# LUMC/kPAL

Hardware: AMD Instinct MI355X
Metric: Gbases/s k-mer counted (k=12, 150bp synthetic) (higher is better)
Workload: dtype int64

## Files before the change

### include/kpal_hip.h

```cpp
#ifndef KPAL_HIP_H
#define KPAL_HIP_H

#include <stddef.h>
#include <stdint.h>

#ifdef __cplusplus
extern "C" {
#endif

#define KPAL_MAX_K 16

#define KPAL_OK 0
#define KPAL_E_INVALID (-1)
#define KPAL_E_NOMEM (-2)
#define KPAL_E_HIP (-3)
#define KPAL_E_STATE (-4)
#define KPAL_E_IO (-5)

#define KPAL_PAIRWISE_PROD 0
#define KPAL_PAIRWISE_SUM 1
#define KPAL_EUCLIDEAN 2

#define KPAL_COSINE 3

// ... 45 lines not shown
int kpal_fastq_flatten(kpal_ctx *ctx, const uint8_t *host_buf, size_t nbytes, const kpal_fastq_options *opt, uint8_t *host_out,
                       uint64_t *n_out);
int kpal_count_records(kpal_ctx *ctx, int k, const uint8_t *host_flat, size_t nbytes, const uint64_t *host_starts,
                       size_t n_records, int64_t *host_out);
int kpal_fasta_records_begin(kpal_ctx *ctx, const uint8_t *host_text, size_t nbytes, uint64_t *n_records, uint64_t *flat_bytes);
int kpal_fasta_records_index(kpal_ctx *ctx, uint64_t *header_off, uint64_t *flat_start);
int kpal_fasta_records_count(kpal_ctx *ctx, int k, uint64_t first, uint64_t n, int64_t *host_out);
int kpal_fasta_records_count_device(kpal_ctx *ctx, int k, uint64_t first, uint64_t n, int64_t *dev_out);
int kpal_fasta_records_file_open(kpal_ctx *ctx, const char *path, uint64_t begin, uint64_t end);
int kpal_fasta_records_file_next(kpal_ctx *ctx, uint64_t *n_records, uint64_t *flat_bytes, uint64_t *text_offset, int *done);
int kpal_fasta_records_file_tell(kpal_ctx *ctx, uint64_t *offset);
int kpal_fasta_records_file_close(kpal_ctx *ctx);
int kpal_count_finish(kpal_ctx *ctx, int64_t *host_out );
int kpal_count_balance(kpal_ctx *ctx);
int kpal_count_last_plan(kpal_ctx *ctx, int *strategy, int *steps1, int *steps2);
#define KPAL_COUNT_STATS 9
int kpal_count_stats(kpal_ctx *ctx, uint64_t *out, int n);
int kpal_count_table(kpal_ctx *ctx, void **dev_table, uint64_t *n_bins);

int kpal_synth_reads_device(kpal_ctx *ctx, uint64_t seed, uint64_t first_read, uint64_t n_reads,
                            int read_len, int noisy, void *dev_out);

#define KPAL_COMM_ID_BYTES 128
int kpal_comm_probe(const char *rccl_library);
int kpal_comm_unique_id(const char *rccl_library, uint8_t *id_out );
int kpal_comm_init(kpal_ctx *ctx, const char *rccl_library, int rank, int world, const uint8_t *id);
int kpal_comm_destroy(kpal_ctx *ctx);
int kpal_comm_reduce_table(kpal_ctx *ctx, int root, int balance);
int kpal_comm_reduce_table_async(kpal_ctx *ctx, int root, int balance);
int kpal_comm_merged_table(kpal_ctx *ctx, void **dev_table, uint64_t *n_bins);
int kpal_comm_reduce_scatter_table(kpal_ctx *ctx, int balance);
// ... 94 lines not shown
```

### kpal_amd/_native.py

```python
import ctypes
import os
import numbers
import threading

import numpy as np

_HERE = os.path.dirname(os.path.abspath(__file__))
LIB_PATH = os.environ.get('KPAL_HIP_LIBRARY', os.path.join(_HERE, 'libkpal_hip.so'))

KPAL_MAX_K = 16
PAIRWISE_PROD, PAIRWISE_SUM, EUCLIDEAN, COSINE = 0, 1, 2, 3
SUMMARY_MIN, SUMMARY_AVERAGE, SUMMARY_MEDIAN = 0, 1, 2
STRATEGY = {'auto': 0, 'global_atomic': 1, 'lds_direct': 2, 'partition': 3, 'partition2': 4, 'partition_chunked': 5, 'partition_quads': 6, 'partition2_quads': 7}

_E_INVALID, _E_NOMEM, _E_HIP, _E_STATE, _E_IO = -1, -2, -3, -4, -5

_lib = None
_lib_lock = threading.Lock()

_vp = ctypes.c_void_p
_i64p = ctypes.POINTER(ctypes.c_int64)
_f64p = ctypes.POINTER(ctypes.c_double)

class DistanceOptions(ctypes.Structure):
# ... 359 lines not shown
        p = _vp()
        n = ctypes.c_uint64(0)
        _check(self._L.kpal_count_table(self._h, ctypes.byref(p), ctypes.byref(n)))
        return p.value, n.value

    def count_balance(self):
        _check(self._L.kpal_count_balance(self._h))

    def count_last_plan(self):
        st, s1, s2 = ctypes.c_int(0), ctypes.c_int(0), ctypes.c_int(0)
        _check(self._L.kpal_count_last_plan(self._h, ctypes.byref(st), ctypes.byref(s1), ctypes.byref(s2)))
        names = {v: n for n, v in STRATEGY.items()}
        return names.get(st.value, str(st.value)), s1.value, s2.value

    def count_stats(self):
        out = (ctypes.c_uint64 * 9)()
        _check(self._L.kpal_count_stats(self._h, out, 9))
        names = ('hot_entries', 'spilled_items', 'unlisted_items', 'fresh_pieces', 'fresh_reruns', 'quad_pieces', 'chunked_pieces', 'split_pieces', 'repeat_pieces')
        return dict(zip(names, (int(v) for v in out)))

    def count_table_view(self):
        ptr, n = self.count_table()
        return DeviceTable(ptr, n, self)

    def synth_reads_device(self, seed, first_read, n_reads, read_len, dev_ptr, noisy=False):
        _check(self._L.kpal_synth_reads_device(self._h, int(seed), int(first_read), int(n_reads), int(read_len),
                                               int(bool(noisy)), _vp(dev_ptr)))

    def count_records(self, k, flat, starts):
        a = np.frombuffer(flat, dtype=np.uint8) if not isinstance(flat, np.ndarray) else np.ascontiguousarray(flat, dtype=np.uint8)
        st = np.ascontiguousarray(starts, dtype=np.uint64)
        n = st.size - 1
        out = np.empty((max(n, 0), 4 ** k), dtype=np.int64)
# ... 312 lines not shown
```

### kpal_amd/csrc/kpal_count.hip

```cpp
#include "kpal_host.hpp"

#include "count_kernels.hpp"
#include "partition_kernels.hpp"
#include "chunk_kernels.hpp"
#include "fasta_kernels.hpp"
#include "fasta_host.hpp"
#include "fastq_kernels.hpp"

#include <cerrno>
#include <fcntl.h>
#include <sys/stat.h>
#include <sys/syscall.h>
#include <unistd.h>

static_assert(sizeof(ChunkPool) <= sizeof(kpal_ctx::chunk_pool_sent), "kpal_ctx::chunk_pool_sent holds a ChunkPool");

static void fq_reset(kpal_ctx *ctx);

KPAL_API int kpal_count_begin(kpal_ctx *ctx, int k)
{
    CTX_ENTER(ctx);
    if (k < 1 || k > KPAL_MAX_K) return set_err(KPAL_E_INVALID, "k=%d out of range 1..%d", k, KPAL_MAX_K);
    if (ctx->merged && (ctx->merged_bins != (1ULL << (2 * k)) || ctx->merged == ctx->table.p)) {
        ctx->merged = nullptr;
// ... 1230 lines not shown
    if (steps1) *steps1 = ctx->plan_steps1;
    if (steps2) *steps2 = ctx->plan_steps2;
    return KPAL_OK;
}

KPAL_API int kpal_count_stats(kpal_ctx *ctx, uint64_t *out, int n)
{
    CTX_ENTER(ctx);
    if (!out || n < 1) return set_err(KPAL_E_INVALID, "out is NULL");
    uint32_t words[4] = {0, 0, 0, 0};
    if (ctx->quad_error_word) {
        HIPCHK(hipMemcpyAsync(words, ctx->quad_error_word, sizeof(words), hipMemcpyDeviceToHost, ctx->stream));
        HIPCHK(hipStreamSynchronize(ctx->stream));
    }
    const uint64_t all[KPAL_COUNT_STATS] = {words[1], words[2], words[3], ctx->stat_fresh_pieces, ctx->stat_fresh_reruns, ctx->stat_quad_pieces,
                                            ctx->stat_chunked_pieces, ctx->stat_split_pieces, ctx->stat_repeat_pieces};
    for (int i = 0; i < n; ++i) out[i] = i < KPAL_COUNT_STATS ? all[i] : 0;
    return KPAL_OK;
}

KPAL_API int kpal_count_table(kpal_ctx *ctx, void **dev_table, uint64_t *n_bins)
{
    if (!ctx) return set_err(KPAL_E_INVALID, "ctx is NULL");
    if (!ctx->counting) return set_err(KPAL_E_STATE, "no count table (call kpal_count_begin)");
    HIPCHK(hipSetDevice(ctx->device));
    CHK(table_ready(ctx));
    if (dev_table) *dev_table = ctx->table.p;
    if (n_bins) *n_bins = ctx->bins;
    return KPAL_OK;
}

// ... 16 lines not shown
```

### kpal_amd/csrc/kpal_ctx.hip

```cpp
#include "kpal_host.hpp"

#include <unistd.h>

static thread_local char g_err[512] = "";

int set_err(int code, const char *fmt, ...)
{
    va_list ap;
    va_start(ap, fmt);
    vsnprintf(g_err, sizeof(g_err), fmt, ap);
    va_end(ap);
    return code;
}

KPAL_API const char *kpal_last_error(void) { return g_err; }
KPAL_API const char *kpal_version(void) { return "kpal_amd 0.4 (gfx950)"; }

int ensure(kpal_ctx *ctx, DevBuf &b, size_t bytes)
{
    if (b.cap >= bytes && b.p) return KPAL_OK;
    if (b.p) {
        HIPCHK(hipStreamSynchronize(ctx->stream));
        HIPCHK(hipFree(b.p));
        b.p = nullptr;
// ... 89 lines not shown
    }
    if (const char *e = getenv("KPAL_BATCH_BYTES")) {
        unsigned long long v = strtoull(e, nullptr, 10);
        if (v >= (1ULL << 20)) {
            ctx->batch_bytes = (size_t)v;
            ctx->batch_bytes_set = true;
        }
    }
    if (const char *e = getenv("KPAL_LEVEL2")) ctx->level2_mode = atoi(e);
    if (const char *e = getenv("KPAL_FASTA_CHUNK")) {
        const unsigned long long v = strtoull(e, nullptr, 10);
        if (v >= 16 && v <= kpal_ctx::kStage) ctx->fa_chunk = (size_t)v;
    }
    if (const char *e = getenv("KPAL_QUAD_STEPS")) ctx->quad_steps_forced = atoi(e);
    if (const char *e = getenv("KPAL_QUAD_STEPS2")) ctx->quad_steps2_forced = atoi(e);
    if (const char *e = getenv("KPAL_QUAD_VERBOSE")) ctx->quad_verbose = atoi(e) != 0;
    if (const char *e = getenv("KPAL_QUAD_REPEAT")) ctx->quad_repeat_forced = atoi(e) != 0 ? 1 : 0;
    if (const char *e = getenv("KPAL_HIST_PACKED")) ctx->quad_hist_unpacked = atoi(e) == 0;
    if (const char *e = getenv("KPAL_DIRECT_SEG")) {
        const long v = atol(e);
        if (v >= 1 && v <= (1 << 20)) {
            ctx->direct_seg = (uint32_t)v;
            ctx->direct_seg_forced = true;
        }
    }
    if (const char *e = getenv("KPAL_SPLIT_ABOVE")) {
        unsigned long long v = strtoull(e, nullptr, 10);
        if (v >= 1024) ctx->split_above = v;
    }
    if (const char *e = getenv("KPAL_QUAD_POOL_MAX")) {
// ... 160 lines not shown
```

### kpal_amd/csrc/kpal_device.hpp

```cpp
#pragma once
#include <hip/hip_runtime.h>
#include <stdint.h>

namespace kpal {

__host__ __device__ inline uint64_t mix64(uint64_t x)
{
    uint64_t z = x + 0x9E3779B97F4A7C15ULL;
    z = (z ^ (z >> 30)) * 0xBF58476D1CE4E5B9ULL;
    z = (z ^ (z >> 27)) * 0x94D049BB133111EBULL;
    return z ^ (z >> 31);
}

__host__ __device__ inline uint64_t revcomp(uint64_t x, int k)
{
    uint64_t y = ~x;
#if defined(__HIP_DEVICE_COMPILE__)
    y = __brevll(y);
#else
    y = ((y >> 1) & 0x5555555555555555ULL) | ((y & 0x5555555555555555ULL) << 1);
    y = ((y >> 2) & 0x3333333333333333ULL) | ((y & 0x3333333333333333ULL) << 2);
    y = ((y >> 4) & 0x0F0F0F0F0F0F0F0FULL) | ((y & 0x0F0F0F0F0F0F0F0FULL) << 4);
    y = ((y >> 8) & 0x00FF00FF00FF00FFULL) | ((y & 0x00FF00FF00FF00FFULL) << 8);
    y = ((y >> 16) & 0x0000FFFF0000FFFFULL) | ((y & 0x0000FFFF0000FFFFULL) << 16);
// ... 174 lines not shown
                                            uint64_t &window, uint32_t &mask, bool edge)
{
    const int lane = threadIdx.x & 63;
    const int64_t c = (int64_t)(step * 64 + lane);
    Chunk cur = encode16(raw);
    if (edge) range_fix(s, c, cur);
    const uint32_t pc = from_left_lane(cur.codes, carry.codes);
    const uint32_t pb = from_left_lane(cur.bad, carry.bad);
    carry.codes = __builtin_amdgcn_readlane(cur.codes, 63);
    carry.bad = __builtin_amdgcn_readlane(cur.bad, 63);
    window = ((uint64_t)pc << 32) | cur.codes;
    mask = emit_mask<K>(pb, cur.bad);
    if (edge) mask &= emit_from_mask(s, c);
}

__device__ __forceinline__ bool interior_steps(const Span &s, uint64_t step0, uint64_t step1)
{
    return step0 * 64 >= 1 && (step0 * 64 - 1) * 16 >= s.lo && step1 * 64 * 16 <= s.hi && s.emit_from <= step0 * 64 * 16;
}

template <int K>
__device__ __forceinline__ void encode_step(const Span &s, uint64_t step, const uint4 raw, Chunk &carry,
                                            uint64_t &window, uint32_t &mask)
{
    encode_step<K>(s, step, raw, carry, window, mask, !interior_steps(s, step, step + 1));
}

__device__ __forceinline__ bool interior_range(const Span &s, uint64_t c0, uint64_t c1)
{
    return c0 >= 1 && (c0 - 1) * 16 >= s.lo && c1 * 16 <= s.hi && s.emit_from <= c0 * 16;
// ... 24 lines not shown
```

### kpal_amd/csrc/kpal_host.hpp

```cpp
#pragma once
#include "../../include/kpal_hip.h"

#include <hip/hip_runtime.h>

#include <algorithm>
#include <cmath>
#include <cstdarg>
#include <cstdio>
#include <cstdlib>
#include <cstring>
#include <string>
#include <thread>
#include <type_traits>
#include <vector>

#include "kpal_device.hpp"
#include "host_pool.hpp"

#define KPAL_API extern "C" __attribute__((visibility("default")))

using namespace kpal;

int set_err(int code, const char *fmt, ...) __attribute__((format(printf, 2, 3)));

// ... 32 lines not shown
    int strategy = KPAL_STRATEGY_AUTO;
    bool counting = false;
    DevBuf table;
    uint64_t bins = 0;
    size_t batch_bytes = (size_t)1 << 30;
    bool batch_bytes_set = false;
    uint64_t split_above = 0xFFFFFFFFull;
    size_t quad_pool_max = (size_t)30 << 30;
    DevBuf keys, cntmat, offs, bucket_start, slice_start;
    DevBuf chunk_meta, chunk_table, chunk_ovf, chunk_sorted;
    DevBuf quad_meta, quad_meta2;
    uint32_t *quad_error_word = nullptr;
    bool chunk_error_armed = false;
    int quad_steps_forced = 0, quad_steps2_forced = 0;
    bool quad_verbose = false;
    int quad_repeat_forced = -1;
    bool sample_hot_rows = false;
    int plan_strategy = 0, plan_steps1 = 0, plan_steps2 = 0;
    uint64_t stat_fresh_pieces = 0, stat_fresh_reruns = 0, stat_quad_pieces = 0, stat_chunked_pieces = 0, stat_split_pieces = 0, stat_repeat_pieces = 0;
    int cached_steps1 = 0, cached_steps2 = 0;
    uint32_t cached_uses = 0;
    size_t cached_bytes = 0;
    bool finalize_pending = false;
    const void *finalize_stage = nullptr;
    bool table_zero_pending = false;
    bool finalize_fresh = false;
    bool fresh_resolved = false;
    bool fresh_feed = false;
    Span fresh_span = {};
    DevBuf direct_list, direct_meta;
    uint32_t direct_seg = 16384;
    uint32_t direct_seg_used = 16384;
    bool quad_hist_unpacked = false;
// ... 190 lines not shown
```

### kpal_amd/csrc/kpal_quads.hip

```cpp
#include "kpal_host.hpp"

#include "quad_kernels.hpp"


double quad_expected_backlog(const std::vector<double> &mu, int slots)
{
    static const double rho_grid[10] = {0.5, 0.6, 0.7, 0.75, 0.8, 0.85, 0.9, 0.925, 0.95, 0.975};
    static const double ratio[4][10] = {
        {1.02, 1.08, 1.25, 1.43, 1.70, 2.19, 3.21, 4.24, 6.34, 12.7},
        {1.00, 1.01, 1.08, 1.17, 1.33, 1.65, 2.34, 3.05, 4.52, 8.9},
        {1.00, 1.00, 1.01, 1.04, 1.12, 1.30, 1.75, 2.24, 3.25, 6.35},
        {1.00, 1.00, 1.00, 1.02, 1.02, 1.10, 1.36, 1.68, 2.37, 4.55}};
    const int ti = slots <= 24 ? 0 : (slots <= 32 ? 1 : (slots <= 64 ? 2 : 3));
    double total = 0.0;
    for (size_t at = 0; at < mu.size();) {
        size_t end = at + 1;
        while (end < mu.size() && mu[end] <= mu[at] * 1.01) ++end;
        const double m = 0.5 * (mu[at] + mu[end - 1]), weight = (double)(end - at);
        at = end;
        if (m <= 0.0) continue;
        const double rho = m / slots;
        if (rho >= 0.995) {
            total += 1e6 * weight;
            continue;
// ... 69 lines not shown
        for (size_t b = 0; b < mu.size(); ++b) mu[b] = per_step[b] * waves * c;
        const double backlog = quad_expected_backlog(mu, slots);
        if (verbose) fprintf(stderr, "[kpal quad] sample: %d steps per wave -> expected backlog %.0f items (fullest row %.1f of %d)\n", c, backlog, mu.back(), slots);
        if (backlog <= budget) {
            *steps_out = c;
            break;
        }
    }
    return KPAL_OK;
}

int launch_partition_quads(kpal_ctx *ctx, const Span &s)
{
    const uint64_t total_steps = (s.nchunks + 63) / 64;
    if (total_steps == 0) return KPAL_OK;
    const int buckets = ctx->k == 12 ? QuadCfg<12>::kBuckets : 512;
    const int slots = ctx->k == 12 ? QuadCfg<12>::kItems : kQuadRowWords / buckets;
    CHK(ensure(ctx, ctx->quad_meta, ((size_t)ctx->num_cu + 4 + 2048 + 512) * sizeof(uint32_t)));
    uint32_t *nrounds = (uint32_t *)ctx->quad_meta.p;
    uint32_t *error = nrounds + ctx->num_cu;
    uint32_t *load = error + 4;
    if (!ctx->quad_error_word) {
        HIPCHK(hipMemsetAsync(error, 0, 4 * sizeof(uint32_t), ctx->stream));
        ctx->quad_error_word = error;
    }
    static const int candidates[] = {8, 7, 6, 4, 3, 2, 1};
    constexpr int waves = 16;
    int steps = 0;
    for (int c : candidates)
        if (c == ctx->quad_steps_forced) steps = c;
// ... 8 lines not shown
        const int rc = quad_choose_steps(ctx, s, load, buckets, slots, waves, candidates, sizeof(candidates) / sizeof(candidates[0]), &steps);
        if (rc != KPAL_OK) return rc;
        repeat = ctx->sample_hot_rows;
        ctx->cached_steps1 = steps;
        ctx->cached_uses = 0;
        ctx->cached_bytes = feed_bytes;
    }
    if (ctx->quad_repeat_forced >= 0) repeat = ctx->quad_repeat_forced != 0;
    if (repeat && steps == 7 && !ctx->quad_steps_forced) steps = 6;
    if (repeat && steps != 7) ++ctx->stat_repeat_pieces;
    ctx->plan_strategy = KPAL_STRATEGY_PARTITION_QUADS;
    ctx->plan_steps1 = steps;
    ctx->plan_steps2 = 0;
    const uint64_t tile_steps = (uint64_t)waves * steps;
    const uint64_t tiles = (total_steps + tile_steps - 1) / tile_steps;
    const uint32_t G = (uint32_t)std::min<uint64_t>((uint64_t)ctx->num_cu, tiles);
    const uint64_t tpb = (tiles + G - 1) / G;
    if (tpb > 0xFFFFFFull) return set_err(KPAL_E_INVALID, "quad partition: batch too large");
    const size_t pool_bytes = (size_t)kQuadRowWords * 4 * G * tpb;
    if (pool_bytes > ctx->quad_pool_max && s.nchunks > 64) return kSplitBatch;
    CHK(ensure(ctx, ctx->keys, pool_bytes));
    uint32_t *pool = (uint32_t *)ctx->keys.p;
    const TableOnly table = {(unsigned long long *)ctx->table.p};
    static const bool allow_staged = [] { const char *e = getenv("KPAL_K12_STAGED"); return !e || atoi(e) != 0; }();
    uint32_t *stage = nullptr;
    if (ctx->k == 12 && allow_staged && (double)feed_bytes <= 240.0 * 4.0 * (double)ctx->bins) {
        CHK(ensure(ctx, ctx->residuals, (size_t)ctx->bins * 4 * sizeof(quad2_stage_t)));
        stage = (uint32_t *)ctx->residuals.p;
    }
#define KPAL_QUAD_LAUNCH(S)                                                                                                  \
    do {                                                                                                                     \
        if (repeat)                                                                                                          \
// ... 37 lines not shown
```

### kpal_amd/csrc/kpal_quads2.hip

```cpp
#include "kpal_host.hpp"

#include "quad_kernels.hpp"

#ifndef KPAL_L1_DEPTH8
#define KPAL_L1_DEPTH8 4
#endif

int launch_partition2_quads(kpal_ctx *ctx, const Span &s, bool fresh)
{
    const uint64_t total_steps = (s.nchunks + 63) / 64;
    if (total_steps == 0) return KPAL_OK;
    const int K = ctx->k;
    const uint32_t NB1 = 1u << (2 * K - 22);
    const uint32_t REP = NB1 >= 256 ? 1u : 256u / NB1;
    const uint32_t S1 = (uint32_t)kQuadRowWords / (NB1 * REP);
    CHK(ensure(ctx, ctx->quad_meta, ((size_t)ctx->num_cu + 4 + 2048 + 512) * sizeof(uint32_t)));
    uint32_t *nrounds1 = (uint32_t *)ctx->quad_meta.p;
    uint32_t *error = nrounds1 + ctx->num_cu;
    if (!ctx->quad_error_word) {
        HIPCHK(hipMemsetAsync(error, 0, 4 * sizeof(uint32_t), ctx->stream));
        ctx->quad_error_word = error;
    }
    static const int candidates[] = {8, 7, 6, 3};
    int steps1 = 0;
    for (int c : candidates)
        if (c == ctx->quad_steps_forced) steps1 = c;
// ... 2 lines not shown
    const bool cached = ctx->cached_steps1 && ctx->cached_steps2 && ctx->cached_uses < 16 && feed_bytes <= 2 * ctx->cached_bytes &&
                        2 * feed_bytes >= ctx->cached_bytes;
    if (cached) {
        if (!steps1) steps1 = ctx->cached_steps1;
        ++ctx->cached_uses;
    } else {
        int chosen = 0;
        const int rc = quad_choose_steps(ctx, s, error + 4, (int)(NB1 * REP), (int)S1, 16, candidates, 4, &chosen, &fine);
        if (rc != KPAL_OK) return rc;
        if (!steps1) steps1 = chosen;
    }
    const bool repeat1 = ctx->quad_repeat_forced >= 0 ? ctx->quad_repeat_forced != 0 : ctx->sample_hot_rows;
    if (repeat1 && steps1 != 7) ++ctx->stat_repeat_pieces;
    const uint64_t tile_steps = 16ull * steps1;
    const uint64_t tiles1 = (total_steps + tile_steps - 1) / tile_steps;
    const uint32_t G1 = (uint32_t)std::min<uint64_t>((uint64_t)std::min(ctx->num_cu, 256), tiles1);
    const uint64_t tpb1 = (tiles1 + G1 - 1) / G1;
    if (tpb1 > 0xFFFFull) return set_err(KPAL_E_INVALID, "quad partition: batch too large");
    const uint64_t per_kib = 1024 / (S1 * 4);
    const uint64_t cap1 = (tpb1 + 1 + per_kib - 1) / per_kib * per_kib;
    if ((size_t)kQuadRowWords * 4 * G1 * cap1 > ctx->quad_pool_max && s.nchunks > 64) return kSplitBatch;
    CHK(ensure(ctx, ctx->residuals, (size_t)kQuadRowWords * 4 * G1 * cap1));
    uint32_t *pool1 = (uint32_t *)ctx->residuals.p;
    const uint32_t units = REP * G1;
    uint32_t G2 = std::max<uint32_t>(1, std::min<uint32_t>(units, (uint32_t)ctx->num_cu * 4 / NB1));
    const uint32_t upw = (units + G2 - 1) / G2;
    G2 = (units + upw - 1) / upw;
    const uint64_t unit_cap = cap1 * S1 * 4;
    if ((uint64_t)upw * unit_cap >= (1ull << 32)) return set_err(KPAL_E_INVALID, "quad partition: batch too large");
    constexpr int kWaves2 = 16;
    int steps2 = 2;
    if (cached) {
        steps2 = ctx->cached_steps2;
    } else {
        double all = 0.0;
        for (double v : fine) all += v;
        const double f1 = std::min(1.0, all * 16.0 * steps1 / (double)kQuadRowWords);
        static const int candidates2[] = {8, 7, 6, 4, 3, 2};
        std::vector<double> mu(fine.size() > 32 ? fine.size() - 32 : 0);
        for (int c : candidates2) {
            for (size_t b = 0; b < mu.size(); ++b) mu[b] = all > 0.0 ? fine[b] / all * (256.0 * f1) * kWaves2 * c : 0.0;
            if (quad_expected_backlog(mu, 64) <= kQuadBacklogMax) {
// ... 150 lines not shown
```

### kpal_amd/csrc/quad_kernels.hpp

```cpp
#pragma once
#include <type_traits>

#include "kpal_device.hpp"
#include "quad2_index.hpp"

namespace kpal {

constexpr int kQuadSpillCap = 2048;
constexpr int kQuadRowWords = 32768;
constexpr int kQuadDummyWords = 4;

template <int K>
struct QuadCfg {
    static_assert(K >= 8 && K <= 16, "quads: k = 8..16");
    static constexpr bool kTwoLevel = K >= 13;
    static constexpr bool kStaged = K >= 12;
    static constexpr int kCoarseBits = kTwoLevel ? 2 * K - 22 : 0;
    static constexpr int kCoarse = 1 << kCoarseBits;
    static constexpr int kRep = kTwoLevel ? (kCoarse >= 256 ? 1 : 256 / kCoarse) : 1;
    static constexpr int kBucketBits = kTwoLevel ? 9 : (K == 12 ? 11 : 9);
    static constexpr int kHistBuckets = 1 << kBucketBits;
    static constexpr int kBuckets = kTwoLevel ? kCoarse * kRep : (1 << kBucketBits);
    static constexpr int kLowBits = kTwoLevel ? 13 : 2 * K - kBucketBits;
    static constexpr int kFormBins = 1 << kLowBits;
// ... 473 lines not shown
                }
            }
        }
    }
    __syncthreads();
    for (int i = threadIdx.x; i < NCNT; i += blockDim.x)
        if (cnt[i]) atomicAdd(&load[i], cnt[i]);
}

__device__ __forceinline__ uint4 fetch_wave_step(const Span &s, uint64_t step, uint32_t lane16)
{
    if ((step + 1) * 64 <= s.nchunks)
        return *reinterpret_cast<const uint4 *>(reinterpret_cast<const char *>(s.base + step * 64) + lane16);
    return fetch_chunk(s, (int64_t)(step * 64 + (lane16 >> 4)));
}


template <int K, int WAVES, int STEPS, int DEPTH, typename SINK = TableOnly, bool REPEAT = false>
__global__ __launch_bounds__(WAVES * 64) void quad_scatter_kernel(Span s, uint64_t tiles_per_block, uint32_t *__restrict__ pool,
                                                                  uint32_t rounds_cap, uint32_t *__restrict__ nrounds,
                                                                  uint32_t *__restrict__ error, SINK sink_arg)
{
    using C = QuadCfg<K>;
    constexpr bool kLists = std::is_same<SINK, TableSink>::value;
    constexpr int S = C::kSlots, NB = C::kBuckets;
    constexpr int THREADS = WAVES * 64;
    constexpr int kQuadTileSteps = WAVES * STEPS;
    constexpr int CARRY = kQuadSpillCap / THREADS;
    constexpr uint32_t CAP = CARRY * THREADS;
    static_assert((WAVES == 8 || WAVES == 16) && STEPS % DEPTH == 0, "tile shape");
// ... 18 lines not shown
        }
        table = TableSinkRef{&sink_lds};
    } else {
        table = sink_arg;
    }
    const int wave = __builtin_amdgcn_readfirstlane((int)(threadIdx.x >> 6)), lane = threadIdx.x & 63;
    const uint32_t lane16 = (uint32_t)lane * 16u;
    for (int i = threadIdx.x; i < kQuadRowWords + kQuadDummyWords; i += THREADS) rows[i] = 0;
    for (int i = threadIdx.x; i < NB; i += THREADS) pos[i] = 0;
    for (int i = threadIdx.x; i < kQuadHotEntries; i += THREADS) hot[i] = QuadHot{0ull, 0u, 0u};
    if (threadIdx.x == 0) {
        spill_cnt[0] = 0;
        spill_cnt[1] = 0;
    }
    __syncthreads();
    const uint64_t total_steps = (s.nchunks + 63) / 64;
    auto tile_step = [&](uint64_t j) -> uint64_t { return ((j * gridDim.x + blockIdx.x) * WAVES + (uint64_t)wave) * STEPS; };
    auto tile_exists = [&](uint64_t j) -> bool { return j < tiles_per_block && (j * gridDim.x + blockIdx.x) * (uint64_t)kQuadTileSteps < total_steps; };
    uint4 raw[DEPTH];
    uint4 rawh;
    {
        const uint64_t f = tile_step(0);
#pragma unroll
        for (int st = 0; st < DEPTH; ++st) raw[st] = fetch_wave_step(s, f + st, lane16);
        rawh = fetch_chunk(s, (int64_t)(f * 64) - 1);
    }
    uint32_t round = 0;
    uint32_t carry_row[CARRY], carry_item[CARRY];
#pragma unroll
    for (int c = 0; c < CARRY; ++c) carry_row[c] = carry_item[c] = 0;
    constexpr int LPR = S / 4;
    constexpr int FI = kQuadRowWords / 4 / THREADS;
    static_assert(THREADS % LPR == 0, "a record is written by one wave");
    uint4 rec[FI];
    bool have_rec = false;
    constexpr int PAIR = C::kPairRows ? 2 : 1;
    static_assert((THREADS / LPR) % PAIR == 0, "row pairs are written by one instruction");
    const uint64_t row_bytes = (uint64_t)gridDim.x * rounds_cap * (uint64_t)(S * 4 * PAIR);
    const uint32_t thread_off = (uint32_t)((uint64_t)(threadIdx.x / (LPR * PAIR)) * row_bytes) + (threadIdx.x % (LPR * PAIR)) * 16u;
    auto store_rec = [&](int i) {
#if defined(KPAL_AB_POOL_FILL)
        if (i % 7 == 6) return;
#endif
        uint32_t o = thread_off;
        asm volatile("" : "+v"(o));
        const uint64_t sc = (uint64_t)(i * (THREADS / (LPR * PAIR))) * row_bytes + ((uint64_t)blockIdx.x * rounds_cap + (round - 1u)) * (uint64_t)(S * 4 * PAIR);
#if defined(KPAL_QUAD_NT)
        uint32_t *q = reinterpret_cast<uint32_t *>(reinterpret_cast<char *>(pool) + sc + o);
        __builtin_nontemporal_store(rec[i].x, q);
        __builtin_nontemporal_store(rec[i].y, q + 1);
        __builtin_nontemporal_store(rec[i].z, q + 2);
        __builtin_nontemporal_store(rec[i].w, q + 3);
#elif defined(KPAL_AB_SCATTER_NO_STORE)
        asm volatile("" ::"v"(rec[i].x ^ rec[i].y ^ rec[i].z ^ rec[i].w), "v"(o), "s"((uint32_t)sc));
#else
        *reinterpret_cast<uint4 *>(reinterpret_cast<char *>(pool) + sc + o) = rec[i];
#endif
    };
    auto store_rec_at = [&](int i, const uint4 &v) {
        const uint64_t sc = (uint64_t)i * (uint64_t)(THREADS / (LPR * PAIR)) * row_bytes + ((uint64_t)blockIdx.x * rounds_cap + (round - 1u)) * (uint64_t)(S * 4 * PAIR);
        *reinterpret_cast<uint4 *>(reinterpret_cast<char *>(pool) + sc + thread_off) = v;
    };
    for (uint64_t j = 0; tile_exists(j); ++j) {
        const uint64_t first = tile_step(j);
        const bool more = tile_exists(j + 1);
        const uint64_t fnext = tile_step(j + 1);
        const bool edge = !interior_steps(s, first, first + STEPS);
        const bool next_inside = more && (fnext + STEPS) * 64 <= s.nchunks;
        uint32_t *spill_n = &spill_cnt[j & 1];
        quad_place_carried<K, CARRY, 1, SINK2, REPEAT>(rows, pos, spill, spill_n, CAP, carry_row, carry_item, table, hot);
        Chunk carry = encode16(rawh);
        range_fix(s, (int64_t)(first * 64) - 1, carry);
        if (more) rawh = fetch_chunk(s, (int64_t)(fnext * 64) - 1);
#pragma unroll
        for (int st = 0; st < STEPS; ++st) {
            uint64_t window;
            uint32_t mask;
            quad_tile_priority<STEPS>(st);
            encode_step<K>(s, first + st, raw[st % DEPTH], carry, window, mask, edge);
            if (have_rec) {
#pragma unroll
                for (int i = st * (FI / STEPS); i < (st + 1) * (FI / STEPS); ++i) store_rec(i);
            }
            {
                uint32_t l16 = lane16;
                asm volatile("" : "+v"(l16));
                if (st + DEPTH < STEPS) raw[st % DEPTH] = fetch_wave_step(s, first + st + DEPTH, l16);
                else if (next_inside) raw[st % DEPTH] = *reinterpret_cast<const uint4 *>(reinterpret_cast<const char *>(s.base + (fnext + (st + DEPTH - STEPS)) * 64) + l16);
                else if (more) raw[st % DEPTH] = fetch_chunk(s, (int64_t)((fnext + (st + DEPTH - STEPS)) * 64 + (l16 >> 4)));
            }
            uint32_t row[4], item[4];
#pragma unroll
            for (int q = 0; q < 4; ++q) {
                const uint64_t x = (window >> (24 - 8 * q)) & C::kXMask;
                quad_split<K>(x, (mask >> (12 - 4 * q)) & 15u, (uint32_t)lane, row[q], item[q]);
            }
            bool place = true;
            if constexpr (REPEAT) {
                if (__builtin_expect(__any(item[1] == item[0] || item[3] == item[2]), 0)) {
                    const bool c01 = item[1] == item[0] && row[1] == row[0] && (item[1] & 15u) == 15u;
                    const bool c23 = item[3] == item[2] && row[3] == row[2] && (item[3] & 15u) == 15u;
                    const unsigned long long cand = __builtin_amdgcn_ballot_w64(c01 || c23);
                    if (cand) {
                        const int src = __ffsll((long long)cand) - 1;
// ... 33 lines not shown
#pragma unroll
            for (int i = 0; i < FI; ++i) {
                const uint4 v = rv[threadIdx.x + (uint32_t)i * THREADS];
                rec[i].x = v.x;
                rec[i].y = v.y;
                rec[i].z = v.z;
                rec[i].w = v.w;
                rv[threadIdx.x + (uint32_t)i * THREADS] = zero4;
            }
            for (int i = threadIdx.x * 4; i < NB; i += THREADS * 4) *reinterpret_cast<uint4 *>(&pos[i]) = zero4;
        }
        if (round >= rounds_cap) {
            if (threadIdx.x == 0) *error = 2u;
        } else {
            have_rec = true;
            ++round;
#pragma unroll
            for (int i = STEPS * (FI / STEPS); i < FI; ++i) store_rec(i);
        }
        lds_barrier();
    }
    if (have_rec) {
#pragma unroll
        for (int i = 0; i < STEPS * (FI / STEPS); ++i) store_rec(i);
    }
    if constexpr (kLists) {
        if (round > 0u && round < rounds_cap) {
            static_assert(!C::kItem3, "plain four-byte slots");
#pragma unroll
            for (int c = 0; c < CARRY; ++c)
                if (carry_item[c]) {
                    const uint32_t off = atomicAdd(&pos[carry_row[c]], 4u);
                    if (off < (uint32_t)S * 4u) {
                        *reinterpret_cast<uint32_t *>(reinterpret_cast<char *>(rows) + carry_row[c] * (uint32_t)(S * 4) + off) = carry_item[c];
                        carry_item[c] = 0;
                    }
                }
            lds_barrier();
            const uint4 *rv = reinterpret_cast<const uint4 *>(rows);
            ++round;
#pragma unroll 1
            for (int h = 0; h < FI; h += 4) {
#pragma unroll
                for (int i = 0; i < 4; ++i) rec[i] = rv[threadIdx.x + (uint32_t)(h + i) * THREADS];
#pragma unroll
                for (int i = 0; i < 4; ++i) store_rec_at(h + i, rec[i]);
            }
        }
    }
    if (threadIdx.x == 0) nrounds[blockIdx.x] = min(round, rounds_cap);
#pragma unroll
    for (int c = 0; c < CARRY; ++c) quad_items_direct_body<K, 1, SINK2>(carry_item[c] != 0u, carry_row[c], carry_item[c], table, hot);
    __syncthreads();
    uint32_t used = 0;
    for (int i = threadIdx.x; i < kQuadHotEntries; i += THREADS) {
// ... 56 lines not shown
    const uint32_t coarse = blockIdx.y;
    for (int i = threadIdx.x; i < kQuadRowWords + kQuadDummyWords; i += THREADS) rows[i] = 0;
    for (int i = threadIdx.x; i < NB; i += THREADS) pos[i] = 0;
    for (int i = threadIdx.x; i < kQuadHotEntries; i += THREADS) hot[i] = QuadHot{0ull, 0u, 0u};
    for (uint32_t i = threadIdx.x; i < 256u; i += THREADS) nr1[i] = i < G1 ? nrounds1[i] : 0u;
    if (threadIdx.x == 0) {
        spill_cnt[0] = 0;
        spill_cnt[1] = 0;
    }
    __syncthreads();
    const uint32_t units = (uint32_t)C1::kRep * G1;
    const uint32_t u0 = blockIdx.x * upw, u1 = min(u0 + upw, units);
    const uint32_t unit_cap = rounds_cap1 * (uint32_t)(S1 * 4);
    const uint32_t stream = (u1 > u0 ? u1 - u0 : 0u) * unit_cap;
    const uint32_t lane16 = (uint32_t)lane * 16u;
    uint64_t nx_p = 0;
    uint32_t nx_g1 = 0, nx_rl = 0, nx_off = 0;
    auto seek = [&](uint64_t j) {
        nx_p = ((j * WAVES + (uint64_t)wave) * STEPS) * 1024ull;
        if (nx_p < (uint64_t)stream) {
            const uint32_t ul = (uint32_t)nx_p / unit_cap;
            nx_off = (uint32_t)nx_p - ul * unit_cap;
            const uint32_t u = u0 + ul;
            nx_rl = u / G1;
            nx_g1 = u - nx_rl * G1;
        }
    };
    auto fetch_next = [&]() -> uint4 {
        uint4 v = make_uint4(0u, 0u, 0u, 0u);
        if (nx_p < (uint64_t)stream) {
            const uint32_t written = nr1[nx_g1] * (uint32_t)(S1 * 4);
            if (nx_off + lane16 < written) {
                const char *src = reinterpret_cast<const char *>(pool1) +
                                  ((uint64_t)((coarse * C1::kRep + nx_rl) * G1 + nx_g1) * rounds_cap1) * (uint64_t)(S1 * 4) + nx_off;
                v = *reinterpret_cast<const uint4 *>(src + lane16);
            }
            nx_p += 1024;
            nx_off += 1024;
            if (nx_off >= unit_cap) {
                nx_off = 0;
                if (++nx_g1 == G1) {
                    nx_g1 = 0;
                    ++nx_rl;
                }
            }
        }
        return v;
    };
    uint4 raw[STEPS];
    seek(0);
#pragma unroll
    for (int st = 0; st < STEPS; ++st) raw[st] = fetch_next();
// ... 10 lines not shown
    bool have_rec = false;
    const uint32_t wg = coarse * gridDim.x + blockIdx.x;
    constexpr uint32_t PIECE = 2u * (uint32_t)kQuadPackedRecordBytes;
    const uint64_t row_bytes = (uint64_t)gridDim.x * rounds_cap2 * (uint64_t)PIECE;
    const uint32_t thread_off = (uint32_t)((uint64_t)(threadIdx.x / (2 * LPR)) * row_bytes) + (threadIdx.x % (2 * LPR)) * 12u;
    auto store_rec = [&](int i) {
        uint32_t o = thread_off;
        asm volatile("" : "+v"(o));
        const uint64_t sc = ((uint64_t)coarse * (NB / 2) + (uint64_t)(i * (THREADS / (2 * LPR)))) * row_bytes + ((uint64_t)blockIdx.x * rounds_cap2 + (round - 1u)) * (uint64_t)PIECE;
        *reinterpret_cast<QuadPacked *>(reinterpret_cast<char *>(pool2) + sc + o) = rec[i];
    };
    auto store_rec_at = [&](int i, const QuadPacked &v) {
        const uint64_t sc = ((uint64_t)coarse * (NB / 2) + (uint64_t)i * (uint64_t)(THREADS / (2 * LPR))) * row_bytes + ((uint64_t)blockIdx.x * rounds_cap2 + (round - 1u)) * (uint64_t)PIECE;
        *reinterpret_cast<QuadPacked *>(reinterpret_cast<char *>(pool2) + sc + thread_off) = v;
    };
    const uint64_t tile_bytes = (uint64_t)WAVES * STEPS * 1024;
    for (uint64_t j = 0; j < tiles_per_block && j * tile_bytes < (uint64_t)stream; ++j) {
        const bool more = j + 1 < tiles_per_block && (j + 1) * tile_bytes < (uint64_t)stream;
        uint32_t *spill_n = &spill_cnt[j & 1];
        quad_place_carried<K, CARRY, 2, TableSinkRef, KM>(rows, pos, spill, spill_n, CAP, carry_row, carry_item, table, hot, coarse);
        if (more) seek(j + 1);
#pragma unroll
        for (int st = 0; st < STEPS; ++st) {
            quad_tile_priority<STEPS>(st);
            const uint4 v = raw[st];
            const uint32_t it[4] = {v.x, v.y, v.z, v.w};
            uint32_t row[4], item[4];
#pragma unroll
            for (int q = 0; q < 4; ++q) {
                const uint32_t t = ((it[q] >> 4) & 8191u) >> 9;
                row[q] = ((it[q] >> 17) & 511u) ^ C::smask(t);
                item[q] = ((it[q] >> 26) << 17) | (it[q] & 0x1FFFFu);
            }
            asm volatile("" ::"v"(row[0]), "v"(item[0]));
            if (have_rec) {
#pragma unroll
// ... 509 lines not shown
```

Measured before the change: 1533.

## Specialise steady-state quad scatter tiles and narrow index math to 32 bits

Result: faster. 1555 (median of 6 runs) (+1.4%).

```diff
diff --git a/include/kpal_hip.h b/include/kpal_hip.h
--- a/include/kpal_hip.h
+++ b/include/kpal_hip.h
@@ -83,7 +83,7 @@
 int kpal_count_finish(kpal_ctx *ctx, int64_t *host_out );
 int kpal_count_balance(kpal_ctx *ctx);
 int kpal_count_last_plan(kpal_ctx *ctx, int *strategy, int *steps1, int *steps2);
-#define KPAL_COUNT_STATS 9
+#define KPAL_COUNT_STATS 11
 int kpal_count_stats(kpal_ctx *ctx, uint64_t *out, int n);
 int kpal_count_table(kpal_ctx *ctx, void **dev_table, uint64_t *n_bins);
 
diff --git a/kpal_amd/_native.py b/kpal_amd/_native.py
--- a/kpal_amd/_native.py
+++ b/kpal_amd/_native.py
@@ -397,9 +397,10 @@
         return names.get(st.value, str(st.value)), s1.value, s2.value
 
     def count_stats(self):
-        out = (ctypes.c_uint64 * 9)()
-        _check(self._L.kpal_count_stats(self._h, out, 9))
-        names = ('hot_entries', 'spilled_items', 'unlisted_items', 'fresh_pieces', 'fresh_reruns', 'quad_pieces', 'chunked_pieces', 'split_pieces', 'repeat_pieces')
+        out = (ctypes.c_uint64 * 11)()
+        _check(self._L.kpal_count_stats(self._h, out, 11))
+        names = ('hot_entries', 'spilled_items', 'unlisted_items', 'fresh_pieces', 'fresh_reruns', 'quad_pieces', 'chunked_pieces', 'split_pieces', 'repeat_pieces',
+                 'scatter_workgroups', 'scatter_workgroups2')
         return dict(zip(names, (int(v) for v in out)))
 
     def count_table_view(self):
diff --git a/kpal_amd/csrc/kpal_count.hip b/kpal_amd/csrc/kpal_count.hip
--- a/kpal_amd/csrc/kpal_count.hip
+++ b/kpal_amd/csrc/kpal_count.hip
@@ -1268,7 +1268,8 @@
         HIPCHK(hipStreamSynchronize(ctx->stream));
     }
     const uint64_t all[KPAL_COUNT_STATS] = {words[1], words[2], words[3], ctx->stat_fresh_pieces, ctx->stat_fresh_reruns, ctx->stat_quad_pieces,
-                                            ctx->stat_chunked_pieces, ctx->stat_split_pieces, ctx->stat_repeat_pieces};
+                                            ctx->stat_chunked_pieces, ctx->stat_split_pieces, ctx->stat_repeat_pieces, ctx->plan_workgroups1,
+                                            ctx->plan_workgroups2};
     for (int i = 0; i < n; ++i) out[i] = i < KPAL_COUNT_STATS ? all[i] : 0;
     return KPAL_OK;
 }
diff --git a/kpal_amd/csrc/kpal_ctx.hip b/kpal_amd/csrc/kpal_ctx.hip
--- a/kpal_amd/csrc/kpal_ctx.hip
+++ b/kpal_amd/csrc/kpal_ctx.hip
@@ -127,6 +127,7 @@
     }
     if (const char *e = getenv("KPAL_QUAD_STEPS")) ctx->quad_steps_forced = atoi(e);
     if (const char *e = getenv("KPAL_QUAD_STEPS2")) ctx->quad_steps2_forced = atoi(e);
+    if (const char *e = getenv("KPAL_QUAD_WORKGROUPS")) ctx->quad_workgroups = std::max(0, atoi(e));
     if (const char *e = getenv("KPAL_QUAD_VERBOSE")) ctx->quad_verbose = atoi(e) != 0;
     if (const char *e = getenv("KPAL_QUAD_REPEAT")) ctx->quad_repeat_forced = atoi(e) != 0 ? 1 : 0;
     if (const char *e = getenv("KPAL_HIST_PACKED")) ctx->quad_hist_unpacked = atoi(e) == 0;
diff --git a/kpal_amd/csrc/kpal_device.hpp b/kpal_amd/csrc/kpal_device.hpp
--- a/kpal_amd/csrc/kpal_device.hpp
+++ b/kpal_amd/csrc/kpal_device.hpp
@@ -212,6 +212,18 @@
     if (edge) mask &= emit_from_mask(s, c);
 }
 
+template <int K>
+__device__ __forceinline__ void encode_step_interior(const uint4 raw, Chunk &carry, uint64_t &window, uint32_t &mask)
+{
+    const Chunk cur = encode16(raw);
+    const uint32_t pc = from_left_lane(cur.codes, carry.codes);
+    const uint32_t pb = from_left_lane(cur.bad, carry.bad);
+    carry.codes = __builtin_amdgcn_readlane(cur.codes, 63);
+    carry.bad = __builtin_amdgcn_readlane(cur.bad, 63);
+    window = ((uint64_t)pc << 32) | cur.codes;
+    mask = emit_mask<K>(pb, cur.bad);
+}
+
 __device__ __forceinline__ bool interior_steps(const Span &s, uint64_t step0, uint64_t step1)
 {
     return step0 * 64 >= 1 && (step0 * 64 - 1) * 16 >= s.lo && step1 * 64 * 16 <= s.hi && s.emit_from <= step0 * 64 * 16;
diff --git a/kpal_amd/csrc/kpal_host.hpp b/kpal_amd/csrc/kpal_host.hpp
--- a/kpal_amd/csrc/kpal_host.hpp
+++ b/kpal_amd/csrc/kpal_host.hpp
@@ -70,9 +70,11 @@
     bool chunk_error_armed = false;
     int quad_steps_forced = 0, quad_steps2_forced = 0;
     bool quad_verbose = false;
+    int quad_workgroups = 0;
     int quad_repeat_forced = -1;
     bool sample_hot_rows = false;
     int plan_strategy = 0, plan_steps1 = 0, plan_steps2 = 0;
+    uint32_t plan_workgroups1 = 0, plan_workgroups2 = 0;
     uint64_t stat_fresh_pieces = 0, stat_fresh_reruns = 0, stat_quad_pieces = 0, stat_chunked_pieces = 0, stat_split_pieces = 0, stat_repeat_pieces = 0;
     int cached_steps1 = 0, cached_steps2 = 0;
     uint32_t cached_uses = 0;
diff --git a/kpal_amd/csrc/kpal_quads.hip b/kpal_amd/csrc/kpal_quads.hip
--- a/kpal_amd/csrc/kpal_quads.hip
+++ b/kpal_amd/csrc/kpal_quads.hip
@@ -107,6 +107,7 @@
 {
     const uint64_t total_steps = (s.nchunks + 63) / 64;
     if (total_steps == 0) return KPAL_OK;
+    if (s.nchunks > kQuadMaxChunks) return kSplitBatch;
     const int buckets = ctx->k == 12 ? QuadCfg<12>::kBuckets : 512;
     const int slots = ctx->k == 12 ? QuadCfg<12>::kItems : kQuadRowWords / buckets;
     CHK(ensure(ctx, ctx->quad_meta, ((size_t)ctx->num_cu + 4 + 2048 + 512) * sizeof(uint32_t)));
@@ -145,8 +146,11 @@
     ctx->plan_steps2 = 0;
     const uint64_t tile_steps = (uint64_t)waves * steps;
     const uint64_t tiles = (total_steps + tile_steps - 1) / tile_steps;
-    const uint32_t G = (uint32_t)std::min<uint64_t>((uint64_t)ctx->num_cu, tiles);
+    uint32_t G = (uint32_t)std::min<uint64_t>((uint64_t)ctx->num_cu, tiles);
+    if (ctx->quad_workgroups > 0) G = std::min(G, (uint32_t)ctx->quad_workgroups);
     const uint64_t tpb = (tiles + G - 1) / G;
+    ctx->plan_workgroups1 = G;
+    ctx->plan_workgroups2 = 0;
     if (tpb > 0xFFFFFFull) return set_err(KPAL_E_INVALID, "quad partition: batch too large");
     const size_t pool_bytes = (size_t)kQuadRowWords * 4 * G * tpb;
     if (pool_bytes > ctx->quad_pool_max && s.nchunks > 64) return kSplitBatch;
diff --git a/kpal_amd/csrc/kpal_quads2.hip b/kpal_amd/csrc/kpal_quads2.hip
--- a/kpal_amd/csrc/kpal_quads2.hip
+++ b/kpal_amd/csrc/kpal_quads2.hip
@@ -10,6 +10,7 @@
 {
     const uint64_t total_steps = (s.nchunks + 63) / 64;
     if (total_steps == 0) return KPAL_OK;
+    if (s.nchunks > kQuadMaxChunks) return kSplitBatch;
     const int K = ctx->k;
     const uint32_t NB1 = 1u << (2 * K - 22);
     const uint32_t REP = NB1 >= 256 ? 1u : 256u / NB1;
@@ -42,7 +43,8 @@
     if (repeat1 && steps1 != 7) ++ctx->stat_repeat_pieces;
     const uint64_t tile_steps = 16ull * steps1;
     const uint64_t tiles1 = (total_steps + tile_steps - 1) / tile_steps;
-    const uint32_t G1 = (uint32_t)std::min<uint64_t>((uint64_t)std::min(ctx->num_cu, 256), tiles1);
+    uint32_t G1 = (uint32_t)std::min<uint64_t>((uint64_t)std::min(ctx->num_cu, 256), tiles1);
+    if (ctx->quad_workgroups > 0) G1 = std::min(G1, (uint32_t)ctx->quad_workgroups);
     const uint64_t tpb1 = (tiles1 + G1 - 1) / G1;
     if (tpb1 > 0xFFFFull) return set_err(KPAL_E_INVALID, "quad partition: batch too large");
     const uint64_t per_kib = 1024 / (S1 * 4);
@@ -52,8 +54,11 @@
     uint32_t *pool1 = (uint32_t *)ctx->residuals.p;
     const uint32_t units = REP * G1;
     uint32_t G2 = std::max<uint32_t>(1, std::min<uint32_t>(units, (uint32_t)ctx->num_cu * 4 / NB1));
+    if (ctx->quad_workgroups > 0) G2 = std::min(G2, (uint32_t)ctx->quad_workgroups);
     const uint32_t upw = (units + G2 - 1) / G2;
     G2 = (units + upw - 1) / upw;
+    ctx->plan_workgroups1 = G1;
+    ctx->plan_workgroups2 = G2;
     const uint64_t unit_cap = cap1 * S1 * 4;
     if ((uint64_t)upw * unit_cap >= (1ull << 32)) return set_err(KPAL_E_INVALID, "quad partition: batch too large");
     constexpr int kWaves2 = 16;
diff --git a/kpal_amd/csrc/quad_kernels.hpp b/kpal_amd/csrc/quad_kernels.hpp
--- a/kpal_amd/csrc/quad_kernels.hpp
+++ b/kpal_amd/csrc/quad_kernels.hpp
@@ -511,6 +511,21 @@
         return *reinterpret_cast<const uint4 *>(reinterpret_cast<const char *>(s.base + step * 64) + lane16);
     return fetch_chunk(s, (int64_t)(step * 64 + (lane16 >> 4)));
 }
+
+__device__ __forceinline__ uint4 fetch_wave_step32(const Span &s, uint32_t nchunks, uint32_t step, uint32_t lane16)
+{
+    if ((step + 1u) * 64u <= nchunks)
+        return *reinterpret_cast<const uint4 *>(reinterpret_cast<const char *>(s.base) + ((uint64_t)step << 10) + lane16);
+    const uint32_t c = step * 64u + (lane16 >> 4);
+    return c < nchunks ? s.base[c] : make_uint4(0u, 0u, 0u, 0u);
+}
+
+__device__ __forceinline__ uint4 fetch_chunk32(const Span &s, uint32_t nchunks, int32_t c)
+{
+    return (uint32_t)c < nchunks ? s.base[(uint32_t)c] : make_uint4(0u, 0u, 0u, 0u);
+}
+
+constexpr uint64_t kQuadMaxChunks = (1ull << 30) + 64;
 
 
 template <int K, int WAVES, int STEPS, int DEPTH, typename SINK = TableOnly, bool REPEAT = false>
@@ -559,16 +574,20 @@
         spill_cnt[1] = 0;
     }
     __syncthreads();
-    const uint64_t total_steps = (s.nchunks + 63) / 64;
-    auto tile_step = [&](uint64_t j) -> uint64_t { return ((j * gridDim.x + blockIdx.x) * WAVES + (uint64_t)wave) * STEPS; };
-    auto tile_exists = [&](uint64_t j) -> bool { return j < tiles_per_block && (j * gridDim.x + blockIdx.x) * (uint64_t)kQuadTileSteps < total_steps; };
+    const uint32_t nch = (uint32_t)s.nchunks;
+    const uint32_t total_steps = (nch + 63u) / 64u;
+    const uint32_t full_chunks = (uint32_t)(s.hi >> 4);
+    const uint32_t emit_chunk = (uint32_t)((s.emit_from + 15u) >> 4);
+    const uint32_t tpb = (uint32_t)tiles_per_block;
+    auto tile_step = [&](uint32_t j) -> uint32_t { return ((j * gridDim.x + blockIdx.x) * (uint32_t)WAVES + (uint32_t)wave) * (uint32_t)STEPS; };
+    auto tile_exists = [&](uint32_t j) -> bool { return j < tpb && (j * gridDim.x + blockIdx.x) * (uint32_t)kQuadTileSteps < total_steps; };
     uint4 raw[DEPTH];
     uint4 rawh;
     {
-        const uint64_t f = tile_step(0);
-#pragma unroll
-        for (int st = 0; st < DEPTH; ++st) raw[st] = fetch_wave_step(s, f + st, lane16);
-        rawh = fetch_chunk(s, (int64_t)(f * 64) - 1);
+        const uint32_t f = tile_step(0);
+#pragma unroll
+        for (int st = 0; st < DEPTH; ++st) raw[st] = fetch_wave_step32(s, nch, f + (uint32_t)st, lane16);
+        rawh = fetch_chunk32(s, nch, (int32_t)(f * 64u) - 1);
     }
     uint32_t round = 0;
     uint32_t carry_row[CARRY], carry_item[CARRY];
@@ -583,15 +602,20 @@
     static_assert((THREADS / LPR) % PAIR == 0, "row pairs are written by one instruction");
     const uint64_t row_bytes = (uint64_t)gridDim.x * rounds_cap * (uint64_t)(S * 4 * PAIR);
     const uint32_t thread_off = (uint32_t)((uint64_t)(threadIdx.x / (LPR * PAIR)) * row_bytes) + (threadIdx.x % (LPR * PAIR)) * 16u;
+    char *rec_at = reinterpret_cast<char *>(pool) + (uint64_t)blockIdx.x * rounds_cap * (uint64_t)(S * 4 * PAIR);
+    auto next_round = [&]() {
+        if (round) rec_at += S * 4 * PAIR;
+        ++round;
+    };
     auto store_rec = [&](int i) {
 #if defined(KPAL_AB_POOL_FILL)
         if (i % 7 == 6) return;
 #endif
         uint32_t o = thread_off;
         asm volatile("" : "+v"(o));
-        const uint64_t sc = (uint64_t)(i * (THREADS / (LPR * PAIR))) * row_bytes + ((uint64_t)blockIdx.x * rounds_cap + (round - 1u)) * (uint64_t)(S * 4 * PAIR);
+        const uint64_t sc = (uint64_t)(i * (THREADS / (LPR * PAIR))) * row_bytes;
 #if defined(KPAL_QUAD_NT)
-        uint32_t *q = reinterpret_cast<uint32_t *>(reinterpret_cast<char *>(pool) + sc + o);
+        uint32_t *q = reinterpret_cast<uint32_t *>(rec_at + sc + o);
         __builtin_nontemporal_store(rec[i].x, q);
         __builtin_nontemporal_store(rec[i].y, q + 1);
         __builtin_nontemporal_store(rec[i].z, q + 2);
@@ -599,40 +623,53 @@
 #elif defined(KPAL_AB_SCATTER_NO_STORE)
         asm volatile("" ::"v"(rec[i].x ^ rec[i].y ^ rec[i].z ^ rec[i].w), "v"(o), "s"((uint32_t)sc));
 #else
-        *reinterpret_cast<uint4 *>(reinterpret_cast<char *>(pool) + sc + o) = rec[i];
+        *reinterpret_cast<uint4 *>(rec_at + sc + o) = rec[i];
 #endif
     };
     auto store_rec_at = [&](int i, const uint4 &v) {
-        const uint64_t sc = (uint64_t)i * (uint64_t)(THREADS / (LPR * PAIR)) * row_bytes + ((uint64_t)blockIdx.x * rounds_cap + (round - 1u)) * (uint64_t)(S * 4 * PAIR);
-        *reinterpret_cast<uint4 *>(reinterpret_cast<char *>(pool) + sc + thread_off) = v;
-    };
-    for (uint64_t j = 0; tile_exists(j); ++j) {
-        const uint64_t first = tile_step(j);
-        const bool more = tile_exists(j + 1);
-        const uint64_t fnext = tile_step(j + 1);
-        const bool edge = !interior_steps(s, first, first + STEPS);
-        const bool next_inside = more && (fnext + STEPS) * 64 <= s.nchunks;
-        uint32_t *spill_n = &spill_cnt[j & 1];
+        const uint64_t sc = (uint64_t)i * (uint64_t)(THREADS / (LPR * PAIR)) * row_bytes;
+        *reinterpret_cast<uint4 *>(rec_at + sc + thread_off) = v;
+    };
+    auto tile = [&](auto steady_tag, const uint32_t j) __attribute__((always_inline)) {
+        constexpr bool STEADY = decltype(steady_tag)::value;
+        const uint32_t first = tile_step(j);
+        const bool more = STEADY || tile_exists(j + 1u);
+        const uint32_t fnext = tile_step(j + 1u);
+        const bool edge = !STEADY && !interior_steps(s, first, first + (uint32_t)STEPS);
+        const bool next_inside = STEADY || (more && (fnext + (uint32_t)STEPS) * 64u <= nch);
+        const char *const in = reinterpret_cast<const char *>(s.base) + ((uint64_t)first << 10);
+        const char *const in_next = reinterpret_cast<const char *>(s.base) + ((uint64_t)fnext << 10);
+        uint32_t *spill_n = &spill_cnt[j & 1u];
         quad_place_carried<K, CARRY, 1, SINK2, REPEAT>(rows, pos, spill, spill_n, CAP, carry_row, carry_item, table, hot);
         Chunk carry = encode16(rawh);
-        range_fix(s, (int64_t)(first * 64) - 1, carry);
-        if (more) rawh = fetch_chunk(s, (int64_t)(fnext * 64) - 1);
+        if constexpr (STEADY) {
+            rawh = *reinterpret_cast<const uint4 *>(in_next - 16);
+        } else {
+            range_fix(s, (int64_t)first * 64 - 1, carry);
+            if (more) rawh = fetch_chunk32(s, nch, (int32_t)(fnext * 64u) - 1);
+        }
 #pragma unroll
         for (int st = 0; st < STEPS; ++st) {
             uint64_t window;
             uint32_t mask;
             quad_tile_priority<STEPS>(st);
-            encode_step<K>(s, first + st, raw[st % DEPTH], carry, window, mask, edge);
-            if (have_rec) {
+            if constexpr (STEADY) encode_step_interior<K>(raw[st % DEPTH], carry, window, mask);
+            else encode_step<K>(s, (uint64_t)(first + (uint32_t)st), raw[st % DEPTH], carry, window, mask, edge);
+            if (STEADY || have_rec) {
 #pragma unroll
                 for (int i = st * (FI / STEPS); i < (st + 1) * (FI / STEPS); ++i) store_rec(i);
             }
             {
                 uint32_t l16 = lane16;
                 asm volatile("" : "+v"(l16));
-                if (st + DEPTH < STEPS) raw[st % DEPTH] = fetch_wave_step(s, first + st + DEPTH, l16);
-                else if (next_inside) raw[st % DEPTH] = *reinterpret_cast<const uint4 *>(reinterpret_cast<const char *>(s.base + (fnext + (st + DEPTH - STEPS)) * 64) + l16);
-                else if (more) raw[st % DEPTH] = fetch_chunk(s, (int64_t)((fnext + (st + DEPTH - STEPS)) * 64 + (l16 >> 4)));
+                if constexpr (STEADY) {
+                    if (st + DEPTH < STEPS) raw[st % DEPTH] = *reinterpret_cast<const uint4 *>(in + (st + DEPTH) * 1024 + l16);
+                    else raw[st % DEPTH] = *reinterpret_cast<const uint4 *>(in_next + (st + DEPTH - STEPS) * 1024 + l16);
+                } else {
+                    if (st + DEPTH < STEPS) raw[st % DEPTH] = fetch_wave_step32(s, nch, first + (uint32_t)(st + DEPTH), l16);
+                    else if (next_inside) raw[st % DEPTH] = *reinterpret_cast<const uint4 *>(in_next + (st + DEPTH - STEPS) * 1024 + l16);
+                    else if (more) raw[st % DEPTH] = fetch_chunk32(s, nch, (int32_t)((fnext + (uint32_t)(st + DEPTH - STEPS)) * 64u + (l16 >> 4)));
+                }
             }
             uint32_t row[4], item[4];
 #pragma unroll
@@ -696,12 +733,21 @@
             if (threadIdx.x == 0) *error = 2u;
         } else {
             have_rec = true;
-            ++round;
+            next_round();
 #pragma unroll
             for (int i = STEPS * (FI / STEPS); i < FI; ++i) store_rec(i);
         }
         lds_barrier();
-    }
+    };
+    auto steady = [&](uint32_t j) -> bool {
+        const uint32_t t0 = (j * gridDim.x + blockIdx.x) * (uint32_t)kQuadTileSteps;
+        const uint32_t t1 = t0 + gridDim.x * (uint32_t)kQuadTileSteps;
+        return j >= 1u && have_rec && j + 1u < tpb && (t1 + (uint32_t)kQuadTileSteps) * 64u <= full_chunks && emit_chunk <= t0 * 64u;
+    };
+    uint32_t j = 0;
+    for (; tile_exists(j) && !steady(j); ++j) tile(std::false_type{}, j);
+    for (; tile_exists(j) && steady(j); ++j) tile(std::true_type{}, j);
+    for (; tile_exists(j); ++j) tile(std::false_type{}, j);
     if (have_rec) {
 #pragma unroll
         for (int i = 0; i < STEPS * (FI / STEPS); ++i) store_rec(i);
@@ -720,7 +766,7 @@
                 }
             lds_barrier();
             const uint4 *rv = reinterpret_cast<const uint4 *>(rows);
-            ++round;
+            next_round();
 #pragma unroll 1
             for (int h = 0; h < FI; h += 4) {
 #pragma unroll
@@ -807,13 +853,14 @@
     const uint32_t unit_cap = rounds_cap1 * (uint32_t)(S1 * 4);
     const uint32_t stream = (u1 > u0 ? u1 - u0 : 0u) * unit_cap;
     const uint32_t lane16 = (uint32_t)lane * 16u;
-    uint64_t nx_p = 0;
+    const uint32_t stream_kib = stream >> 10;
+    uint32_t nx_p = 0;
     uint32_t nx_g1 = 0, nx_rl = 0, nx_off = 0;
-    auto seek = [&](uint64_t j) {
-        nx_p = ((j * WAVES + (uint64_t)wave) * STEPS) * 1024ull;
-        if (nx_p < (uint64_t)stream) {
-            const uint32_t ul = (uint32_t)nx_p / unit_cap;
-            nx_off = (uint32_t)nx_p - ul * unit_cap;
+    auto seek = [&](uint32_t j) {
+        nx_p = (j * (uint32_t)WAVES + (uint32_t)wave) * (uint32_t)STEPS;
+        if (nx_p < stream_kib) {
+            const uint32_t ul = (nx_p << 10) / unit_cap;
+            nx_off = (nx_p << 10) - ul * unit_cap;
             const uint32_t u = u0 + ul;
             nx_rl = u / G1;
             nx_g1 = u - nx_rl * G1;
@@ -821,14 +868,14 @@
     };
     auto fetch_next = [&]() -> uint4 {
         uint4 v = make_uint4(0u, 0u, 0u, 0u);
-        if (nx_p < (uint64_t)stream) {
+        if (nx_p < stream_kib) {
             const uint32_t written = nr1[nx_g1] * (uint32_t)(S1 * 4);
             if (nx_off + lane16 < written) {
                 const char *src = reinterpret_cast<const char *>(pool1) +
                                   ((uint64_t)((coarse * C1::kRep + nx_rl) * G1 + nx_g1) * rounds_cap1) * (uint64_t)(S1 * 4) + nx_off;
                 v = *reinterpret_cast<const uint4 *>(src + lane16);
             }
-            nx_p += 1024;
+            nx_p += 1u;
             nx_off += 1024;
             if (nx_off >= unit_cap) {
                 nx_off = 0;
@@ -869,12 +916,12 @@
         const uint64_t sc = ((uint64_t)coarse * (NB / 2) + (uint64_t)i * (uint64_t)(THREADS / (2 * LPR))) * row_bytes + ((uint64_t)blockIdx.x * rounds_cap2 + (round - 1u)) * (uint64_t)PIECE;
         *reinterpret_cast<QuadPacked *>(reinterpret_cast<char *>(pool2) + sc + thread_off) = v;
     };
-    const uint64_t tile_bytes = (uint64_t)WAVES * STEPS * 1024;
-    for (uint64_t j = 0; j < tiles_per_block && j * tile_bytes < (uint64_t)stream; ++j) {
-        const bool more = j + 1 < tiles_per_block && (j + 1) * tile_bytes < (uint64_t)stream;
-        uint32_t *spill_n = &spill_cnt[j & 1];
+    constexpr uint32_t kTileKib = (uint32_t)(WAVES * STEPS);
+    for (uint32_t j = 0; j < tiles_per_block && j * kTileKib < stream_kib; ++j) {
+        const bool more = j + 1u < tiles_per_block && (j + 1u) * kTileKib < stream_kib;
+        uint32_t *spill_n = &spill_cnt[j & 1u];
         quad_place_carried<K, CARRY, 2, TableSinkRef, KM>(rows, pos, spill, spill_n, CAP, carry_row, carry_item, table, hot, coarse);
-        if (more) seek(j + 1);
+        if (more) seek(j + 1u);
 #pragma unroll
         for (int st = 0; st < STEPS; ++st) {
             quad_tile_priority<STEPS>(st);
```
